# eth-ait/MultiPly

Measured on NVIDIA H100. Metric: rays/sec, higher is better.
Workload: dtype f32 (fp16 hi/lo split tensor-core operands, fp32 accumulate)

## Files before the change

multiply_b200/csrc/mlp_tc.cu:

```cuda
#include "common.cuh"
#include <vector>
#include <mutex>
#include <type_traits>
#include <stdlib.h>

namespace mp {

enum {
  K_SP_PLAIN = 0,
  K_SP_SAVE = 1,
  K_SP_SEED = 2,
  K_FEAT = 3,
  K_BWD = 4,
  K_FINAL_GRAD = 5,
  K_RELU = 6
};
enum {
  F_INJECT_EMB = 1,
  F_SDF_DOT = 2,
  F_SKIP_GRAD = 4,
  F_EXTRA_IN = 8,
  F_RGB_OUT = 16
};
constexpr int kMaxSteps = 24;
constexpr int kSlotBytes = 32768;
constexpr int kRing = 3;
constexpr int kBlobSlots = 170;

struct TcStep {
  int nk;
  int kind;
  int flags;
  int sig;
  const float* bias;
  int slot_off;
  int sc;
  int terms;
};

struct TcProgram {
  int nsteps;
  TcStep step[kMaxSteps];
  const uint4* blob;
  const float* inv_scale;
  int d_in, multires, E, inj_col, n_extra;
  const float* w8row;
  const float* b8;
  const float* Wrgb;
  const float* brgb;
};

struct TcIO : MlpCall {
  float rz;
  char* scratch;
  size_t scratch_per_cta;
};

constexpr int kConsumers = 2;
constexpr int kThreads = 128 * (1 + kConsumers);

constexpr size_t kSigBytes = (size_t)8 * kConsumers * 32 * 128 * 16;
constexpr size_t kFeatBytes = (size_t)kConsumers * 32 * 128 * 16;
constexpr size_t kGeBytes = (size_t)96 * 128 * 4;
constexpr size_t kEmbBytes = (size_t)96 * 128 * 4;
constexpr size_t kScratchPerCta = kSigBytes + kFeatBytes + kGeBytes + kEmbBytes;

constexpr int kABytes = 2 * 4 * 128 * 128;
constexpr int kSmemBytes = kABytes + kRing * kSlotBytes + 256 + 1024;
static_assert(kSmemBytes <= 232448, "shared memory budget of one CTA (227 KB)");

__device__ __forceinline__ uint32_t smem_u32(const void* p) { return (uint32_t)__cvta_generic_to_shared(p); }

__device__ __forceinline__ void mbar_init(uint64_t* bar, uint32_t count) {
  asm volatile("mbarrier.init.shared::cta.b64 [%0], %1;" ::"r"(smem_u32(bar)), "r"(count));
}
__device__ __forceinline__ void mbar_arrive(uint64_t* bar) {
  asm volatile("mbarrier.arrive.shared::cta.b64 _, [%0];" ::"r"(smem_u32(bar)) : "memory");
}
__device__ __forceinline__ void mbar_expect_tx(uint64_t* bar, uint32_t bytes) {
  asm volatile("mbarrier.arrive.expect_tx.shared::cta.b64 _, [%0], %1;" ::"r"(smem_u32(bar)), "r"(bytes) : "memory");
}
__device__ __forceinline__ void mbar_wait(uint64_t* bar, uint32_t parity) {
  asm volatile(
      "{\n"
      ".reg .pred p;\n"
      "WAIT_LOOP:\n"
      "mbarrier.try_wait.parity.shared::cta.b64 p, [%0], %1;\n"
      "@p bra WAIT_DONE;\n"
      "bra WAIT_LOOP;\n"
      "WAIT_DONE:\n"
      "}\n" ::"r"(smem_u32(bar)),
      "r"(parity)
      : "memory");
}
__device__ __forceinline__ void bulk_g2s(void* dst, const void* src, uint32_t bytes, uint64_t* bar) {
  asm volatile("cp.async.bulk.shared::cluster.global.mbarrier::complete_tx::bytes [%0], [%1], %2, [%3];" ::"r"(
                   smem_u32(dst)),
               "l"(src), "r"(bytes), "r"(smem_u32(bar))
               : "memory");
}
__device__ __forceinline__ void prefetch_l2(const void* p, uint32_t bytes) {
  asm volatile("cp.async.bulk.prefetch.L2.global [%0], %1;" ::"l"(p), "r"(bytes) : "memory");
}
__device__ __forceinline__ void fence_async_smem() { asm volatile("fence.proxy.async.shared::cta;" ::: "memory"); }

__device__ __forceinline__ void wg_sync(int id) { asm volatile("bar.sync %0, 128;" ::"r"(id) : "memory"); }

__device__ __forceinline__ void wgmma_fence() { asm volatile("wgmma.fence.sync.aligned;" ::: "memory"); }
__device__ __forceinline__ void wgmma_commit() { asm volatile("wgmma.commit_group.sync.aligned;" ::: "memory"); }
template <int N>
__device__ __forceinline__ void wgmma_wait() {
  asm volatile("wgmma.wait_group.sync.aligned %0;" ::"n"(N) : "memory");
}
__device__ __forceinline__ void acc_fence(float* d) {
#pragma unroll
  for (int i = 0; i < 128; ++i) asm volatile("" : "+f"(d[i])::"memory");
}

#define MP_D4(i) "+f"(d[i]), "+f"(d[i + 1]), "+f"(d[i + 2]), "+f"(d[i + 3])
#define MP_D16(i) MP_D4(i), MP_D4(i + 4), MP_D4(i + 8), MP_D4(i + 12)
__device__ __forceinline__ void wgmma_f16(float* d, uint64_t a_desc, uint64_t b_desc, uint32_t accumulate) {
  asm volatile(
      "{\n"
      ".reg .pred p;\n"
      "setp.ne.b32 p, %130, 0;\n"
      "wgmma.mma_async.sync.aligned.m64n256k16.f32.f16.f16 "
      "{%0, %1, %2, %3, %4, %5, %6, %7, %8, %9, %10, %11, %12, %13, %14, %15, "
      "%16, %17, %18, %19, %20, %21, %22, %23, %24, %25, %26, %27, %28, %29, %30, %31, "
      "%32, %33, %34, %35, %36, %37, %38, %39, %40, %41, %42, %43, %44, %45, %46, %47, "
      "%48, %49, %50, %51, %52, %53, %54, %55, %56, %57, %58, %59, %60, %61, %62, %63, "
      "%64, %65, %66, %67, %68, %69, %70, %71, %72, %73, %74, %75, %76, %77, %78, %79, "
      "%80, %81, %82, %83, %84, %85, %86, %87, %88, %89, %90, %91, %92, %93, %94, %95, "
      "%96, %97, %98, %99, %100, %101, %102, %103, %104, %105, %106, %107, %108, %109, %110, %111, "
      "%112, %113, %114, %115, %116, %117, %118, %119, %120, %121, %122, %123, %124, %125, %126, %127}, "
      "%128, %129, p, 1, 1, 0, 0;\n"
      "}\n"
      : MP_D16(0), MP_D16(16), MP_D16(32), MP_D16(48), MP_D16(64), MP_D16(80), MP_D16(96), MP_D16(112)
      : "l"(a_desc), "l"(b_desc), "r"(accumulate));
}
#undef MP_D16
#undef MP_D4

__device__ __forceinline__ uint64_t make_desc(uint32_t saddr) {
  return (uint64_t)((saddr >> 4) & 0x3FFF) | (1ull << 16) | ((uint64_t)(1024 >> 4) << 32) | (1ull << 62);
}

__device__ __forceinline__ uint32_t a_off(int row, int kb, int ch) {
  return (uint32_t)(kb * 16384 + row * 128 + ((ch ^ (row & 7)) << 4));
}

__device__ __forceinline__ void split2(float a, float b, uint32_t& hi, uint32_t& lo) {
  __half2 h = __floats2half2_rn(a, b);
  float2 f = __half22float2(h);
  __half2 l = __floats2half2_rn(a - f.x, b - f.y);
  hi = *(uint32_t*)&h;
  lo = *(uint32_t*)&l;
}
__device__ __forceinline__ void split8(const float* v, uint4& hi, uint4& lo) {
  split2(v[0], v[1], hi.x, lo.x);
  split2(v[2], v[3], hi.y, lo.y);
  split2(v[4], v[5], hi.z, lo.z);
  split2(v[6], v[7], hi.w, lo.w);
}

__device__ __forceinline__ void sts128(uint32_t A32, uint32_t off, const uint4& v) {
  asm volatile("st.shared.v4.b32 [%0], {%1, %2, %3, %4};" ::"r"(A32 + off), "r"(v.x), "r"(v.y), "r"(v.z), "r"(v.w));
}
__device__ __forceinline__ void store_a8(uint32_t A32, int row, int col, const float* v) {
  uint4 hi, lo;
  split8(v, hi, lo);
  uint32_t o = a_off(row, col >> 6, (col >> 3) & 7);
  sts128(A32, o, hi);
  sts128(A32, 65536 + o, lo);
}
__device__ __forceinline__ void stsm4(uint32_t addr, uint32_t a, uint32_t b, uint32_t c, uint32_t e) {
  asm volatile("stmatrix.sync.aligned.m8n8.x4.shared.b16 [%0], {%1, %2, %3, %4};" ::"r"(addr), "r"(a), "r"(b), "r"(c),
               "r"(e));
}
__device__ __forceinline__ void store_pairs(uint32_t lane_base, uint32_t lane_x, int jp, const uint4& hi, const uint4& lo) {
  const uint32_t addr = lane_base + (uint32_t)(jp >> 2) * 16384u + ((((uint32_t)(2 * jp) & 7u) ^ lane_x) << 4);
  stsm4(addr, hi.x, hi.y, hi.z, hi.w);
  stsm4(addr + 65536u, lo.x, lo.y, lo.z, lo.w);
}
__device__ __forceinline__ void store_acc16(uint32_t lane_base, uint32_t lane_x, int jp, const float* v) {
  uint4 hi, lo;
  split8(v, hi, lo);
  store_pairs(lane_base, lane_x, jp, hi, lo);
}

__device__ __forceinline__ float quad_sum(float v) {
  v += __shfl_xor_sync(0xffffffffu, v, 1);
  v += __shfl_xor_sync(0xffffffffu, v, 2);
  return v;
}

__device__ __forceinline__ float4 ld_stream(const float4* p) {
  float4 v;
  asm volatile("ld.global.cg.v4.f32 {%0,%1,%2,%3}, [%4];" : "=f"(v.x), "=f"(v.y), "=f"(v.z), "=f"(v.w) : "l"(p));
  return v;
}
__device__ __forceinline__ uint4 ld_stream(const uint4* p) {
  uint4 v;
  asm volatile("ld.global.cg.v4.u32 {%0,%1,%2,%3}, [%4];" : "=r"(v.x), "=r"(v.y), "=r"(v.z), "=r"(v.w) : "l"(p));
  return v;
}
__device__ __forceinline__ void st_stream(float4* p, const float4& v) {
  asm volatile("st.global.cg.v4.f32 [%0], {%1,%2,%3,%4};" ::"l"(p), "f"(v.x), "f"(v.y), "f"(v.z), "f"(v.w) : "memory");
}
__device__ __forceinline__ void st_stream(uint4* p, const uint4& v) {
  asm volatile("st.global.cg.v4.u32 [%0], {%1,%2,%3,%4};" ::"l"(p), "r"(v.x), "r"(v.y), "r"(v.z), "r"(v.w) : "memory");
}

__device__ __forceinline__ void discard_line(const void* p, float dep) {
  asm volatile("discard.global.L2 [%0], 128;" ::"l"(p), "f"(dep) : "memory");
}
__device__ __forceinline__ void discard_line(const void* p, uint32_t dep) {
  asm volatile("discard.global.L2 [%0], 128;" ::"l"(p), "r"(dep) : "memory");
}

__device__ __forceinline__ float ex2_approx(float x) {
  float y;
  asm("ex2.approx.ftz.f32 %0, %1;" : "=f"(y) : "f"(x));
  return y;
}
__device__ __forceinline__ float lg2_approx(float x) {
  float y;
  asm("lg2.approx.ftz.f32 %0, %1;" : "=f"(y) : "f"(x));
  return y;
}
__device__ __forceinline__ float rcp_approx(float x) {
  float y;
  asm("rcp.approx.ftz.f32 %0, %1;" : "=f"(y) : "f"(x));
  return y;
}
__device__ __forceinline__ float softplus_fast(float z) {
  float t = z * 144.26950408889634f;
  float u = ex2_approx(t);
  float y = lg2_approx(1.f + u) * 0.0069314718055994531f;
  return t > 28.853900817779268f ? z : y;
}
__device__ __forceinline__ void softplus_fast_grad(float z, float& y, float& d) {
  float t = z * 144.26950408889634f;
  float u = ex2_approx(t);
  float w = 1.f + u;
  float r = rcp_approx(w);
  float ys = lg2_approx(w) * 0.0069314718055994531f;
  bool big = t > 28.853900817779268f;
  y = big ? z : ys;
  d = big ? 1.f : u * r;
}

__device__ __forceinline__ void final_grad(const TcProgram& P, const TcIO& io, const float* acc, float isc, int q,
                                           const float* ge, const float* emb, const int (&rowt)[2],
                                           const bool (&valid)[2], const int (&pt)[2], const int (&slot)[2],
                                           float (&nrm)[2][3]) {
  const int d = P.d_in;
  float gax[2][4] = {{0.f, 0.f, 0.f, 0.f}, {0.f, 0.f, 0.f, 0.f}};
  const int nterm = 1 + 2 * P.multires;
#pragma unroll
  for (int j = 0; j < 8; ++j) {
    if (j < 2 * d) {
      const int a = j >> 1;
#pragma unroll
      for (int e = 0; e < 4; ++e) {
        const int jj = (8 * j + 2 * q + (e & 1)) & 15;
        if (jj < nterm) {
          const int h = e >> 1;
          const int fq = (jj - 1) >> 1;
          const bool is_cos = ((jj - 1) & 1) != 0;
          const int k = (jj == 0) ? a : d + 2 * fq * d + (is_cos ? d : 0) + a;
          const float pg = ge[(size_t)k * 128 + rowt[h]];
          const float tot = fmaf(acc[4 * j + e], isc, pg);
          float w = 1.f;
          if (jj > 0) {
            const float pe = emb[(size_t)(is_cos ? k - d : k + d) * 128 + rowt[h]];
            w = (float)(1 << fq) * (is_cos ? -pe : pe);
          }
          gax[h][a] = fmaf(w, tot, gax[h][a]);
        }
      }
    }
  }
#pragma unroll
  for (int h = 0; h < 2; ++h) {
#pragma unroll
    for (int a = 0; a < 4; ++a) gax[h][a] = quad_sum(gax[h][a]);
    const float gx0 = gax[h][0], gx1 = d > 1 ? gax[h][1] : 0.f, gx2 = d > 2 ? gax[h][2] : 0.f;
    if (q == 0 && io.grad && valid[h]) {
      io.grad[3 * (size_t)pt[h]] = gx0;
      io.grad[3 * (size_t)pt[h] + 1] = gx1;
      io.grad[3 * (size_t)pt[h] + 2] = gx2;
    }
    float n0 = 0.f, n1 = 0.f, n2 = 0.f;
    if (io.jinv && valid[h]) {
      const float4* J4 = (const float4*)(io.jinv + 12 * (size_t)pt[h]);
      const float4 ja = __ldg(J4), jb = __ldg(J4 + 1), jc = __ldg(J4 + 2);
      float v0 = gx0 * ja.x + gx1 * ja.w + gx2 * jb.z;
      float v1 = gx0 * ja.y + gx1 * jb.x + gx2 * jb.w;
      float v2 = gx0 * ja.z + gx1 * jb.y + gx2 * jc.x;
      float nr = fmaxf(sqrtf(v0 * v0 + v1 * v1 + v2 * v2), 1e-12f);
      const float inr = 1.f / nr;
      v0 *= inr; v1 *= inr; v2 *= inr;
      float n2r = fmaxf(sqrtf(v0 * v0 + v1 * v1 + v2 * v2), 1e-6f);
      const float in2 = 1.f / n2r;
      n0 = v0 * in2; n1 = v1 * in2; n2 = v2 * in2;
      if (q == 0 && io.nrm) {
        io.nrm[3 * (size_t)slot[h]] = n0;
        io.nrm[3 * (size_t)slot[h] + 1] = n1;
        io.nrm[3 * (size_t)slot[h] + 2] = n2;
      }
    }
    nrm[h][0] = n0;
    nrm[h][1] = n1;
    nrm[h][2] = n2;
  }
}

__global__ void __launch_bounds__(kThreads, 1) tc_chain_kernel(const __grid_constant__ TcProgram P,
                                                               const __grid_constant__ TcIO io) {
  extern __shared__ uint8_t smem_raw[];
  const int warp = threadIdx.x >> 5, lane = threadIdx.x & 31;
  char* base = (char*)(((uintptr_t)smem_raw + 1023) & ~(uintptr_t)1023);
  char* A = base;
  const uint32_t A32 = smem_u32(A);
  char* ring = base + kABytes;
  uint64_t* bars = (uint64_t*)(ring + kRing * kSlotBytes);
  uint64_t* full = bars;
  uint64_t* empty = bars + kRing;

  const int count = io.count ? min(io.cap, *io.count) : io.cap;
  const int ntiles = (count + 127) >> 7;

  if (threadIdx.x == 0) {
    for (int i = 0; i < kRing; ++i) {
      mbar_init(&full[i], 1);
      mbar_init(&empty[i], 4 * kConsumers);
    }
    asm volatile("fence.mbarrier_init.release.cluster;" ::: "memory");
  }
  __syncthreads();

  if (warp < 4) {
    asm volatile("setmaxnreg.dec.sync.aligned.u32 40;\n" ::: "memory");
    if (warp == 0 && lane == 0) {
      uint32_t it = 0;
      for (int tile = blockIdx.x; tile < ntiles; tile += gridDim.x) {
        for (int s = 0; s < P.nsteps; ++s) {
          const char* src = (const char*)P.blob + (size_t)P.step[s].slot_off * kSlotBytes;
          const int nslot = 2 * P.step[s].nk;
          const int jstep = P.step[s].terms == 1 ? 2 : 1;
          for (int j = 0; j < nslot; j += jstep, ++it) {
            int r = it % kRing;
            uint32_t ph = (it / kRing) & 1;
            mbar_wait(&empty[r], ph ^ 1);
            mbar_expect_tx(&full[r], kSlotBytes);
            bulk_g2s(ring + (size_t)r * kSlotBytes, src + (size_t)j * kSlotBytes, kSlotBytes, &full[r]);
          }
        }
      }
    }
    return;
  }
  asm volatile("setmaxnreg.inc.sync.aligned.u32 232;\n" ::: "memory");
  const int g = (warp >> 2) - 1;
  const int t = threadIdx.x & 127;
  const int wq = warp & 3, q = lane & 3;
  const int bar_id = 1 + g;
  int rowt[2];
  rowt[0] = 64 * g + 16 * wq + (lane >> 2);
  rowt[1] = rowt[0] + 8;
  const int mi = lane >> 3, rr = lane & 7;
  const uint32_t lane_base = A32 + (uint32_t)(64 * g + 16 * wq + 8 * (mi & 1) + rr) * 128u;
  const uint32_t lane_x = (uint32_t)((mi >> 1) ^ rr);
  const uint32_t a_hi = A32 + (uint32_t)g * 8192u, a_lo = a_hi + 65536u;

  char* scr = io.scratch + (size_t)blockIdx.x * io.scratch_per_cta;
  float4* sig = (float4*)scr;
  uint4* fsc = (uint4*)(scr + kSigBytes) + (size_t)g * 32 * 128;
  float* ge = (float*)(scr + kSigBytes + kFeatBytes);
  float* emb = (float*)(scr + kSigBytes + kFeatBytes + kGeBytes);
  const int d = P.d_in, E = P.E;

  float acc[128];
#pragma unroll
  for (int i = 0; i < 128; ++i) acc[i] = 0.f;
  uint32_t it = 0;

  for (int tile = blockIdx.x; tile < ntiles; tile += gridDim.x) {
    int pt[2], slot[2];
    bool valid[2];
    float x[2][4];
#pragma unroll
    for (int h = 0; h < 2; ++h) {
      pt[h] = tile * 128 + rowt[h];
      valid[h] = pt[h] < count;
      for (int a = 0; a < 4; ++a) x[h][a] = 0.f;
      if (valid[h])
        for (int a = 0; a < d; ++a) x[h][a] = io.x[(size_t)pt[h] * d + a];
      slot[h] = valid[h] ? (io.slot ? io.slot[pt[h]] : pt[h]) : 0;
    }
    {
      const int npair = d * P.multires;
      for (int pi = q; pi < npair; pi += 4) {
        const int f = pi / d, a = pi - f * d;
#pragma unroll
        for (int h = 0; h < 2; ++h) {
          float sn, cs;
          sincosf(__fmul_rn(x[h][a], (float)(1 << f)), &sn, &cs);
          emb[(size_t)(d + 2 * f * d + a) * 128 + rowt[h]] = sn;
          emb[(size_t)(d + (2 * f + 1) * d + a) * 128 + rowt[h]] = cs;
        }
      }
      if (q == 0)
        for (int a = 0; a < d; ++a)
#pragma unroll
          for (int h = 0; h < 2; ++h) emb[(size_t)a * 128 + rowt[h]] = x[h][a];
      if (io.dirs) {
        float dv[2][3];
#pragma unroll
        for (int h = 0; h < 2; ++h)
          for (int a = 0; a < 3; ++a) dv[h][a] = valid[h] ? io.dirs[(size_t)pt[h] * 3 + a] : 0.f;
        const int nvp = (P.n_extra - 3) / 2;
        for (int pi = q; pi < nvp; pi += 4) {
          const int f = pi / 3, a = pi - f * 3;
#pragma unroll
          for (int h = 0; h < 2; ++h) {
            float sn, cs;
            sincosf(__fmul_rn(dv[h][a], (float)(1 << f)), &sn, &cs);
            ge[(size_t)(3 + 6 * f + a) * 128 + rowt[h]] = sn;
            ge[(size_t)(3 + 6 * f + 3 + a) * 128 + rowt[h]] = cs;
          }
        }
        if (q == 0)
          for (int a = 0; a < 3; ++a)
#pragma unroll
            for (int h = 0; h < 2; ++h) ge[(size_t)a * 128 + rowt[h]] = dv[h][a];
      }
      __threadfence_block();
      wg_sync(bar_id);
      const int njp = P.step[0].nk * 4;
      for (int jp = 0; jp < njp; ++jp) {
        float v[8];
#pragma unroll
        for (int i = 0; i < 8; ++i) {
          const int c = 16 * jp + 8 * (i >> 2) + 2 * q + (i & 1);
          v[i] = (c < E) ? emb[(size_t)c * 128 + rowt[(i >> 1) & 1]] : 0.f;
        }
        store_acc16(lane_base, lane_x, jp, v);
      }
    }
    float nrm[2][3] = {{0.f, 0.f, 0.f}, {0.f, 0.f, 0.f}};
    for (int s = 0; s < P.nsteps; ++s) {
      const TcStep st = P.step[s];
      const float isc = P.inv_scale[st.sc] * fmaf(io.rz, (float)(4 * st.nk * (st.terms == 1 ? 1 : 3)), 1.f);
      const bool one_term = st.terms == 1;
      if (t == 0) {
        char* ws = io.scratch + (size_t)blockIdx.x * io.scratch_per_cta;
        if (st.kind == K_BWD && st.sig >= 0)
          prefetch_l2(ws + (((size_t)st.sig * kConsumers + g) * 32 * 128) * 16, 32 * 128 * 16);
        if (st.kind == K_FINAL_GRAD) prefetch_l2(ws + kSigBytes + (size_t)g * 32 * 128 * 16, 32 * 128 * 16);
      }

      fence_async_smem();
      wg_sync(bar_id);
      wgmma_fence();
      bool held = false;
      uint32_t held_slot = 0;
      auto release = [&](uint32_t slot_it) {
        if (lane == 0) mbar_arrive(&empty[slot_it % kRing]);
      };
      auto slot_issued = [&](uint32_t slot_it) {
        wgmma_commit();
        if (held) {
          wgmma_wait<1>();
          release(held_slot);
        }
        held = true;
        held_slot = slot_it;
      };
      for (int kc = 0; kc < st.nk; ++kc) {
        if (kc == 4) {
          wgmma_wait<0>();
          acc_fence(acc);
          if (held) release(held_slot);
          held = false;
#pragma unroll
          for (int h = 0; h < 2; ++h) {
#pragma unroll
            for (int c8 = 0; c8 < 16; c8 += 8) {
              const int e0 = 16 * q + c8;
              float xv[8];
#pragma unroll
              for (int j = 0; j < 8; ++j) xv[j] = 0.f;
              if (io.dirs) {
#pragma unroll
                for (int j = 0; j < 8; ++j)
                  if (e0 + j < P.n_extra) xv[j] = ge[(size_t)(e0 + j) * 128 + rowt[h]];
              } else if (e0 == 0) {
                xv[0] = x[h][0]; xv[1] = x[h][1]; xv[2] = x[h][2];
                xv[3] = nrm[h][0]; xv[4] = nrm[h][1]; xv[5] = nrm[h][2];
              }
              store_a8(A32, rowt[h], e0, xv);
            }
          }
          fence_async_smem();
          wg_sync(bar_id);
          wgmma_fence();
        }
        const uint32_t ka = (uint32_t)(kc & 3) * 16384u;
        int r = it % kRing;
        mbar_wait(&full[r], (it / kRing) & 1);
        uint32_t wb = smem_u32(ring + (size_t)r * kSlotBytes);
#pragma unroll
        for (int ks = 0; ks < 4; ++ks) {
          const uint64_t bd = make_desc(wb + ks * 32);
          wgmma_f16(acc, make_desc(a_hi + ka + ks * 32), bd, (kc | ks) != 0);
          if (!one_term) wgmma_f16(acc, make_desc(a_lo + ka + ks * 32), bd, 1);
        }
        slot_issued(it++);
        if (!one_term) {
          r = it % kRing;
          mbar_wait(&full[r], (it / kRing) & 1);
          wb = smem_u32(ring + (size_t)r * kSlotBytes);
#pragma unroll
          for (int ks = 0; ks < 4; ++ks) wgmma_f16(acc, make_desc(a_hi + ka + ks * 32), make_desc(wb + ks * 32), 1);
          slot_issued(it++);
        }
      }
      wgmma_wait<0>();
      acc_fence(acc);
      if (held) release(held_slot);

      auto reload_features = [&]() {
#pragma unroll
        for (int jp = 0; jp < 16; ++jp) {
          const uint4 fh = ld_stream(&fsc[(size_t)jp * 128 + t]);
          const uint4 fl = ld_stream(&fsc[(size_t)(16 + jp) * 128 + t]);
          store_pairs(lane_base, lane_x, jp, fh, fl);
          if ((lane & 7) == 0) {
            discard_line(&fsc[(size_t)jp * 128 + t], fh.x);
            discard_line(&fsc[(size_t)(16 + jp) * 128 + t], fl.x);
          }
        }
      };
      if (st.kind == K_FINAL_GRAD) {
        final_grad(P, io, acc, isc, q, ge, emb, rowt, valid, pt, slot, nrm);
        if (s + 1 < P.nsteps) reload_features();
        continue;
      }

      auto run_epi = [&](auto kind) {
        constexpr int KIND = decltype(kind)::value;
        float dot[2][3] = {{0.f, 0.f, 0.f}, {0.f, 0.f, 0.f}};
#pragma unroll
        for (int jp = 0; jp < 16; ++jp) {
          float* v = acc + 8 * jp;
          float yv[8];
#pragma unroll
          for (int jj = 0; jj < 2; ++jj) {
            const int j = 2 * jp + jj;
            const int c = 8 * j + 2 * q;
            float* u = v + 4 * jj;
            float b[2] = {0.f, 0.f};
            if constexpr (KIND != K_BWD) {
              const float2 b2 = __ldg((const float2*)(st.bias + c));
              b[0] = b2.x;
              b[1] = b2.y;
            }
            if constexpr (KIND == K_SP_SEED) {
              const float2 w2 = __ldg((const float2*)(P.w8row + c));
              const float w[2] = {w2.x, w2.y};
#pragma unroll
              for (int e = 0; e < 4; ++e) {
                float y, dd;
                softplus_fast_grad(fmaf(u[e], isc, b[e & 1]), y, dd);
                dot[e >> 1][0] = fmaf(y, w[e & 1], dot[e >> 1][0]);
                yv[4 * jj + e] = y;
                u[e] = dd * w[e & 1];
              }
            } else if constexpr (KIND == K_SP_SAVE || KIND == K_SP_PLAIN) {
              if constexpr (KIND == K_SP_SAVE) {
                float dd[4];
#pragma unroll
                for (int e = 0; e < 4; ++e) softplus_fast_grad(fmaf(u[e], isc, b[e & 1]), u[e], dd[e]);
                st_stream(&sig[(((size_t)st.sig * kConsumers + g) * 32 + j) * 128 + t], make_float4(dd[0], dd[1], dd[2], dd[3]));
              } else {
#pragma unroll
                for (int e = 0; e < 4; ++e) u[e] = softplus_fast(fmaf(u[e], isc, b[e & 1]));
              }
              if ((st.flags & F_INJECT_EMB) && c + 1 >= P.inj_col) {
#pragma unroll
                for (int e = 0; e < 4; ++e)
                  if (c + (e & 1) >= P.inj_col) u[e] = emb[(size_t)(c + (e & 1) - P.inj_col) * 128 + rowt[e >> 1]];
              }
              if (st.flags & F_SDF_DOT) {
                const float2 w2 = __ldg((const float2*)(P.w8row + c));
                dot[0][0] = fmaf(u[0], w2.x, fmaf(u[1], w2.y, dot[0][0]));
                dot[1][0] = fmaf(u[2], w2.x, fmaf(u[3], w2.y, dot[1][0]));
              }
            } else if constexpr (KIND == K_FEAT) {
#pragma unroll
              for (int e = 0; e < 4; ++e) u[e] = fmaf(u[e], isc, b[e & 1]);
              if (io.feat) {
#pragma unroll
                for (int h = 0; h < 2; ++h)
                  if (valid[h]) *(float2*)(io.feat + (size_t)pt[h] * 256 + c) = make_float2(u[2 * h], u[2 * h + 1]);
              }
            } else if constexpr (KIND == K_BWD) {
              float4 s4 = make_float4(1.f, 1.f, 1.f, 1.f);
              const float4* sp = &sig[(((size_t)(st.sig < 0 ? 0 : st.sig) * kConsumers + g) * 32 + j) * 128 + t];
              if (st.sig >= 0) s4 = ld_stream(sp);
              const float sv[4] = {s4.x, s4.y, s4.z, s4.w};
              if ((st.flags & F_SKIP_GRAD) && c + 1 >= P.inj_col) {
#pragma unroll
                for (int e = 0; e < 4; ++e) {
                  const float gval = u[e] * isc;
                  const int col = c + (e & 1);
                  if (col >= P.inj_col) {
                    ge[(size_t)(col - P.inj_col) * 128 + rowt[e >> 1]] = gval;
                    u[e] = 0.f;
                  } else {
                    u[e] = gval * sv[e];
                  }
                }
              } else {
#pragma unroll
                for (int e = 0; e < 4; ++e) u[e] *= isc * sv[e];
              }
              if (st.sig >= 0 && (lane & 7) == 0) discard_line(sp, s4.x);
            } else {
#pragma unroll
              for (int e = 0; e < 4; ++e) u[e] = fmaxf(fmaf(u[e], isc, b[e & 1]), 0.f);
              if (st.flags & F_RGB_OUT) {
#pragma unroll
                for (int k = 0; k < 3; ++k) {
                  const float2 w2 = __ldg((const float2*)(P.Wrgb + 256 * k + c));
                  dot[0][k] = fmaf(u[0], w2.x, fmaf(u[1], w2.y, dot[0][k]));
                  dot[1][k] = fmaf(u[2], w2.x, fmaf(u[3], w2.y, dot[1][k]));
                }
              }
            }
          }
          if constexpr (KIND == K_SP_SEED) {
            uint4 fh, fl;
            split8(yv, fh, fl);
            st_stream(&fsc[(size_t)jp * 128 + t], fh);
            st_stream(&fsc[(size_t)(16 + jp) * 128 + t], fl);
          }
          bool to_a = true;
          if constexpr (KIND == K_RELU) to_a = !(st.flags & F_RGB_OUT);
          if (to_a) store_acc16(lane_base, lane_x, jp, v);
        }
        if (st.flags & F_SDF_DOT) {
#pragma unroll
          for (int h = 0; h < 2; ++h) {
            const float sdot = quad_sum(dot[h][0]);
            if (q == 0 && valid[h] && io.sdf) io.sdf[slot[h]] = __ldg(P.b8) + sdot;
          }
        }
        if constexpr (KIND == K_RELU) {
          if (st.flags & F_RGB_OUT) {
#pragma unroll
            for (int h = 0; h < 2; ++h) {
#pragma unroll
              for (int k = 0; k < 3; ++k) {
                const float z = __ldg(P.brgb + k) + quad_sum(dot[h][k]);
                if (q == 0 && valid[h] && io.rgb) io.rgb[3 * (size_t)slot[h] + k] = 1.f / (1.f + __expf(-z));
              }
            }
          }
        }
      };
      switch (st.kind) {
        case K_SP_PLAIN: run_epi(std::integral_constant<int, K_SP_PLAIN>{}); break;
        case K_SP_SAVE: run_epi(std::integral_constant<int, K_SP_SAVE>{}); break;
        case K_SP_SEED: run_epi(std::integral_constant<int, K_SP_SEED>{}); break;
        case K_FEAT: run_epi(std::integral_constant<int, K_FEAT>{}); break;
        case K_BWD: run_epi(std::integral_constant<int, K_BWD>{}); break;
        default: run_epi(std::integral_constant<int, K_RELU>{}); break;
      }
      if (st.flags & F_SKIP_GRAD) __threadfence_block();
    }
  }
}

struct TcBlob {
  TcProgram sdf_prog;
  TcProgram full_prog;
  TcProgram fwd_prog;
  bool has_full;
};

__global__ void absmax_kernel(const float* __restrict__ W, int n, float* __restrict__ inv_scale) {
  __shared__ float s[256];
  float m = 0.f;
  for (int i = threadIdx.x; i < n; i += blockDim.x) m = fmaxf(m, fabsf(W[i]));
  s[threadIdx.x] = m;
  __syncthreads();
  for (int o = 128; o > 0; o >>= 1) {
    if (threadIdx.x < o) s[threadIdx.x] = fmaxf(s[threadIdx.x], s[threadIdx.x + o]);
    __syncthreads();
  }
  if (threadIdx.x == 0) {
    float mx = s[0];
    int ex = 0;
    if (mx > 0.f) frexpf(mx, &ex);
    float sc = ldexpf(1.f, 14 - ex);
    inv_scale[0] = 1.f / sc;
  }
}

__global__ void pack_slot_kernel(const float* __restrict__ W, int ld, int transposed, int n_off, int k_off,
                                 int n_valid, int k_valid, int kc, const float* __restrict__ inv_scale,
                                 uint8_t* __restrict__ dst_hi, uint8_t* __restrict__ dst_lo, int perm16) {
  int idx = blockIdx.x * blockDim.x + threadIdx.x;
  if (idx >= 256 * 64) return;
  int n = idx >> 6, k = idx & 63;
  int kk = kc * 64 + k;
  int ns = n;
  if (perm16) {
    const int dd = perm16, a = n >> 4, j = n & 15;
    ns = n_valid;
    if (n < 64 && a < dd) {
      const int k = (j == 0) ? a : dd + ((j - 1) >> 1) * 2 * dd + ((j - 1) & 1) * dd + a;
      if (k < n_valid) ns = k;
    }
  }
  float w = 0.f;
  if (ns < n_valid && kk < k_valid)
    w = transposed ? W[(size_t)(k_off + kk) * ld + n_off + ns] : W[(size_t)(n_off + ns) * ld + k_off + kk];
  w = __fdiv_rn(w, inv_scale[0]);
  __half h = __float2half_rn(w);
  __half l = __float2half_rn(w - __half2float(h));
  uint32_t off = (uint32_t)(n * 128 + ((((k >> 3) ^ (n & 7))) << 4) + (k & 7) * 2);
  *(__half*)(dst_hi + off) = h;
  *(__half*)(dst_lo + off) = l;
}

__global__ void copy_strided_kernel(const float* __restrict__ src, int stride, int n, float* __restrict__ dst) {
  int i = blockIdx.x * blockDim.x + threadIdx.x;
  if (i < n) dst[i] = src[(size_t)i * stride];
}

__global__ void pad_rows_kernel(const float* __restrict__ src, int lds, int nrows, int ncols, float* __restrict__ dst) {
  int i = blockIdx.x * blockDim.x + threadIdx.x;
  if (i >= nrows * 256) return;
  int r = i >> 8, c = i & 255;
  dst[i] = (c < ncols) ? src[(size_t)r * lds + c] : 0.f;
}

__global__ void fold_mm_kernel(const float* __restrict__ Wc, int ldc, int coff, const float* __restrict__ W8f, int ld8,
                               const float* __restrict__ b8f, int n_rows, float* __restrict__ M, int ldm,
                               float* __restrict__ cb) {
  int k = blockIdx.x * 16 + threadIdx.x, n = blockIdx.y * 16 + threadIdx.y;
  if (n >= n_rows || k >= 256) return;
  const float* w = Wc + (size_t)n * ldc + coff;
  double acc = 0.0;
  for (int j = 0; j < 256; ++j) acc += (double)w[j] * (double)W8f[(size_t)j * ld8 + k];
  M[(size_t)n * ldm + k] = (float)acc;
  if (k == 0) {
    double a2 = 0.0;
    for (int j = 0; j < 256; ++j) a2 += (double)w[j] * (double)b8f[j];
    cb[n] = (float)a2;
  }
}

__global__ void fill_extra_cols_kernel(const float* __restrict__ Wt, int n_out, int n_extra, float* __restrict__ M, int ldm) {
  int i = blockIdx.x * blockDim.x + threadIdx.x;
  if (i >= 256 * 64) return;
  int n = i >> 6, e = i & 63;
  M[(size_t)n * ldm + 256 + e] = (n < n_out && e < n_extra) ? Wt[(size_t)e * n_out + n] : 0.f;
}

size_t tc_pack_bytes() { return (size_t)kBlobSlots * kSlotBytes + (1 << 20); }

struct PackCtx {
  cudaStream_t st;
  uint8_t* blob;
  int nslots;
  int nlayers;
  float* inv_scale;
};

static int pack_layer(PackCtx& c, TcStep& stp, int kind, int flags, int sig, const float* bias, const float* W, int ld,
                      int transposed, int n_off, int n_valid, int k_valid, int nk, int total_elems, int perm16 = 0) {
  MP_REQUIRE(c.nslots + 2 * nk <= kBlobSlots, "tc_pack: slot budget exceeded (%d)", c.nslots + 2 * nk);
  const int layer = c.nlayers++;
  stp.nk = nk;
  stp.kind = kind;
  stp.flags = flags;
  stp.sig = sig;
  stp.bias = bias;
  stp.slot_off = c.nslots;
  stp.sc = layer;
  stp.terms = 3;
  absmax_kernel<<<1, 256, 0, c.st>>>(W, total_elems, c.inv_scale + layer);
  MP_LAUNCH_CHECK();
  for (int kc = 0; kc < nk; ++kc) {
    uint8_t* hi = c.blob + (size_t)c.nslots * kSlotBytes;
    uint8_t* lo = hi + kSlotBytes;
    pack_slot_kernel<<<64, 256, 0, c.st>>>(W, ld, transposed, n_off, 0, n_valid, k_valid, kc, c.inv_scale + layer, hi,
                                           lo, perm16);
    MP_LAUNCH_CHECK();
    c.nslots += 2;
  }
  return 0;
}

void tc_free(Field& f) {
  delete (TcBlob*)f.tc;
  f.tc = nullptr;
}

int tc_pack(Field& f, Arena& a, cudaStream_t st) {
  TcBlob* tb = new TcBlob();
  memset(tb, 0, sizeof(*tb));
  f.tc = tb;
  const int E = f.emb_dim;
  PackCtx c;
  c.st = st;
  c.nslots = 0;
  c.nlayers = 0;
  c.blob = (uint8_t*)a.take<uint4>((size_t)kBlobSlots * kSlotBytes / 16);
  c.inv_scale = a.take<float>(32);
  float* w8row = a.take<float>(256);
  float* Wrgb = a.take<float>(3 * 256);
  float* b8feat = a.take<float>(256);
  MP_REQUIRE(a.ok, "tc_pack: storage too small");
  MP_CHECK_CUDA(cudaMemsetAsync(c.blob, 0, (size_t)kBlobSlots * kSlotBytes, st));
  TcProgram P;
  memset(&P, 0, sizeof(P));
  P.blob = (const uint4*)c.blob;
  P.inv_scale = c.inv_scale;
  P.d_in = f.d_in;
  P.multires = f.multires;
  P.E = E;
  P.inj_col = kHidden - E;
  P.w8row = w8row;
  P.b8 = f.imp_b[8];
  P.Wrgb = Wrgb;
  P.n_extra = f.ren_extra;
  copy_strided_kernel<<<1, 256, 0, st>>>(f.imp_W[8], 1, 256, w8row);
  MP_LAUNCH_CHECK();
  copy_strided_kernel<<<1, 256, 0, st>>>(f.imp_b[8] + 1, 1, 256, b8feat);
  MP_LAUNCH_CHECK();
  int s = 0;
  for (int l = 0; l < 8; ++l) {
    const int in = f.imp_in[l], out = f.imp_out[l];
    const int flags = ((l == f.skip_layer - 1) ? F_INJECT_EMB : 0) | ((l == 7) ? F_SDF_DOT : 0);
    MP_TRY(pack_layer(c, P.step[s++], K_SP_PLAIN, flags, l, (l == 0) ? f.imp_b0_eff : f.imp_b[l], f.imp_W[l], in, 0,
                      0, out, (l == 0) ? E : in, (l == 0) ? (E + 63) / 64 : 4, out * in));
  }
  P.nsteps = s;
  tb->sdf_prog = P;
  tb->fwd_prog = P;
  MP_TRY(pack_layer(c, tb->fwd_prog.step[s], K_FEAT, 0, -1, b8feat, f.imp_W[8], 256, 0, 1, 256, 256, 4, 257 * 256));
  tb->fwd_prog.nsteps = s + 1;
  const bool fg_chain = (f.ren_mode == 0) && (f.n_ren == 5) && f.ren_out[0] == 256;
  const bool bg_chain = (f.ren_mode == 1) && (f.n_ren == 2) && f.ren_out[0] <= 256 && f.ren_extra <= 27;
  tb->has_full = fg_chain || bg_chain;
  constexpr int kLdM = 320;
  float* Mfold = a.take<float>(256 * kLdM);
  f.ren_cb = a.take<float>(264);
  f.ren_b0_fold = a.take<float>(264);
  MP_REQUIRE(a.ok, "tc_pack: storage too small");
  if (tb->has_full) {
    const int in0 = f.ren_in[0] == 0 ? 0 : (f.ren_mode == 0 ? 6 + 8 + 256 : f.ren_extra + 32 + 256);
    const int coff = f.ren_mode == 0 ? 14 : f.ren_extra + 32;
    const int o0 = f.ren_out[0];
    fold_mm_kernel<<<dim3(256 / 16, div_up(o0, 16)), dim3(16, 16), 0, st>>>(f.ren_W[0], in0, coff, f.imp_W[8] + 256, 256,
                                                                          f.imp_b[8] + 1, o0, Mfold, kLdM, f.ren_cb);
    MP_LAUNCH_CHECK();
    MP_REQUIRE(f.ren_extra <= 64, "tc_pack: more than 64 extra colour inputs");
    fill_extra_cols_kernel<<<64, 256, 0, st>>>(f.ren_Wt[0], o0, f.ren_extra, Mfold, kLdM);
    MP_LAUNCH_CHECK();
  }
  if (bg_chain) {
    const int o0 = f.ren_out[0];
    MP_TRY(pack_layer(c, P.step[s++], K_RELU, F_EXTRA_IN | F_RGB_OUT, -1, f.ren_b0_fold, Mfold, kLdM, 0, 0, o0, kLdM, 5,
                      256 * kLdM));
    pad_rows_kernel<<<div_up(3 * 256, 256), 256, 0, st>>>(f.ren_W[1], o0, 3, o0, Wrgb);
    MP_LAUNCH_CHECK();
    P.brgb = f.ren_b[1];
    P.nsteps = s;
    tb->full_prog = P;
  }
  if (fg_chain) {
    for (int l = 0; l < 8; ++l) P.step[l].kind = (l == 7) ? K_SP_SEED : K_SP_SAVE;
    for (int l = 7; l >= 1; --l) {
      const int in = f.imp_in[l], out = f.imp_out[l];
      MP_TRY(pack_layer(c, P.step[s++], K_BWD, (l == f.skip_layer) ? F_SKIP_GRAD : 0, l - 1, nullptr, f.imp_W[l], in, 1,
                        0, in, out, 4, out * in));
    }
    MP_REQUIRE(f.d_in <= 4 && 1 + 2 * f.multires <= 14,
               "tc_pack: the final-gradient step keeps 1 + 2 * multires <= 14 embedding columns per axis");
    MP_TRY(pack_layer(c, P.step[s++], K_FINAL_GRAD, 0, -1, nullptr, f.imp_W[0], f.imp_in[0], 1, 0, E, 256, 4,
                      256 * f.imp_in[0], f.d_in));
    MP_TRY(pack_layer(c, P.step[s++], K_RELU, F_EXTRA_IN, -1, f.ren_b0_fold, Mfold, kLdM, 0, 0, 256, kLdM, 5,
                      256 * kLdM));
    for (int l = 1; l < 4; ++l)
      MP_TRY(pack_layer(c, P.step[s++], K_RELU, (l == 3) ? F_RGB_OUT : 0, -1, f.ren_b[l], f.ren_W[l], 256, 0, 0, 256,
                        256, 4, 256 * 256));
    MP_CHECK_CUDA(cudaMemcpyAsync(Wrgb, f.ren_W[4], (size_t)3 * 256 * sizeof(float), cudaMemcpyDeviceToDevice, st));
    P.brgb = f.ren_b[4];
    P.nsteps = s;
    tb->full_prog = P;
  }
  return 0;
}

size_t tc_workspace_bytes(int N) { return (size_t)sm_count() * kScratchPerCta + 4096; }

struct ProfEntry {
  cudaEvent_t e0, e1;
  int kind;
  int cap;
  int* host_count;
};
static std::mutex g_prof_mu;
static std::atomic<bool> g_prof_on{false};
static std::vector<ProfEntry>* g_prof = nullptr;
static int* g_prof_pinned = nullptr;
static int g_prof_used = 0;
constexpr int kProfMax = 1 << 16;

int prof_enable(int on) {
  std::lock_guard<std::mutex> g(g_prof_mu);
  if (on && !g_prof) {
    g_prof = new std::vector<ProfEntry>();
    MP_CHECK_CUDA(cudaMallocHost(&g_prof_pinned, kProfMax * sizeof(int)));
  }
  g_prof_on = on != 0;
  return 0;
}
int prof_read(double* ms, long long* launches, double* points, int reset) {
  for (int k = 0; k < 4; ++k) {
    ms[k] = 0;
    launches[k] = 0;
    points[k] = 0;
  }
  std::lock_guard<std::mutex> g(g_prof_mu);
  if (!g_prof) return 0;
  for (auto& e : *g_prof) {
    MP_CHECK_CUDA(cudaEventSynchronize(e.e1));
    float t = 0.f;
    MP_CHECK_CUDA(cudaEventElapsedTime(&t, e.e0, e.e1));
    ms[e.kind] += t;
    launches[e.kind] += 1;
    int n = e.host_count ? *e.host_count : e.cap;
    points[e.kind] += (double)(n < e.cap ? n : e.cap);
  }
  if (reset) {
    for (auto& e : *g_prof) {
      cudaEventDestroy(e.e0);
      cudaEventDestroy(e.e1);
    }
    g_prof->clear();
    g_prof_used = 0;
  }
  return 0;
}

std::atomic<int> g_precision{0};

constexpr float kRzPerMma = 1.72e-8f;

static int tc_launch(const TcProgram& P0, TcIO io, void* ws, size_t ws_bytes, cudaStream_t st, MlpProg kind) {
  TcProgram P = P0;
  {
    const int mode = g_precision.load();
    for (int s = 0; s < P.nsteps; ++s)
      P.step[s].terms = (mode == 2 || (mode == 1 && P.step[s].kind == K_RELU)) ? 1 : 3;
  }
  int grid = sm_count();
  {
    static int grid_override = -1;
    if (grid_override < 0) {
      const char* eg = getenv("MP_TC_GRID");
      grid_override = eg ? atoi(eg) : 0;
    }
    if (grid_override > 0 && grid_override < grid) grid = grid_override;
  }
  int maxtiles = (io.cap + 127) / 128;
  if (grid > maxtiles) grid = maxtiles;
  if (grid < 1) return 0;
  MP_REQUIRE(ws && ws_bytes >= (size_t)grid * kScratchPerCta, "tensor-core engine: workspace too small (%zu < %zu)",
             ws_bytes, (size_t)grid * kScratchPerCta);
  io.scratch = (char*)ws;
  io.scratch_per_cta = kScratchPerCta;
  static const float rz_scale = [] {
    const char* er = getenv("MP_TC_RZ_SCALE");
    return er ? (float)atof(er) : 1.f;
  }();
  io.rz = kRzPerMma * rz_scale;
  {
    static std::mutex attr_mu;
    static unsigned long long attr_done = 0;
    int dev = 0;
    MP_CHECK_CUDA(cudaGetDevice(&dev));
    std::lock_guard<std::mutex> g(attr_mu);
    if (dev < 0 || dev >= 64 || !((attr_done >> dev) & 1ull)) {
      MP_CHECK_CUDA(cudaFuncSetAttribute(tc_chain_kernel, cudaFuncAttributeMaxDynamicSharedMemorySize, kSmemBytes));
      if (dev >= 0 && dev < 64) attr_done |= 1ull << dev;
    }
  }
  ProfEntry pe;
  std::unique_lock<std::mutex> prof_lock(g_prof_mu, std::defer_lock);
  if (g_prof_on.load()) prof_lock.lock();
  const bool prof = prof_lock.owns_lock() && g_prof_on.load() && g_prof && g_prof_used < kProfMax;
  if (prof) {
    MP_CHECK_CUDA(cudaEventCreate(&pe.e0));
    MP_CHECK_CUDA(cudaEventCreate(&pe.e1));
    pe.kind = (int)kind;
    pe.cap = io.cap;
    pe.host_count = nullptr;
    if (io.count) {
      pe.host_count = g_prof_pinned + g_prof_used++;
      MP_CHECK_CUDA(cudaMemcpyAsync(pe.host_count, io.count, sizeof(int), cudaMemcpyDeviceToHost, st));
    }
    MP_CHECK_CUDA(cudaEventRecord(pe.e0, st));
  }
  tc_chain_kernel<<<grid, kThreads, kSmemBytes, st>>>(P, io);
  MP_LAUNCH_CHECK();
  if (prof) {
    MP_CHECK_CUDA(cudaEventRecord(pe.e1, st));
    g_prof->push_back(pe);
  }
  return 0;
}

int tc_run(const Field& f, const MlpCall& c, void* ws, size_t ws_bytes, cudaStream_t st) {
  MP_REQUIRE(f.tc, "tensor-core engine: field not packed");
  const TcBlob& tb = *(const TcBlob*)f.tc;
  const MlpProg prog = mlp_prog(c);
  TcIO io{};
  static_cast<MlpCall&>(io) = c;
  if (prog == MlpProg::kSdf) return tc_launch(tb.sdf_prog, io, ws, ws_bytes, st, prog);
  if (prog == MlpProg::kForward) return tc_launch(tb.fwd_prog, io, ws, ws_bytes, st, prog);
  if (prog == MlpProg::kBg) {
    MP_REQUIRE(tb.has_full && f.ren_mode == 1, "tensor-core engine: not a background field");
    return tc_launch(tb.full_prog, io, ws, ws_bytes, st, prog);
  }
  MP_REQUIRE(tb.has_full, "tensor-core engine: this field has no fused shading program");
  if (c.feat) {
    TcIO fio{};
    fio.x = c.x;
    fio.slot = c.slot;
    fio.count = c.count;
    fio.cap = c.cap;
    fio.feat = c.feat;
    MP_TRY(tc_launch(tb.fwd_prog, fio, ws, ws_bytes, st, MlpProg::kForward));
    io.feat = nullptr;
  }
  return tc_launch(tb.full_prog, io, ws, ws_bytes, st, prog);
}

}
```

Before: 446,900.

## Split weight slots into 32-wide K halves with 64B swizzle and deeper ring

Halves each TMA weight slot to 16KB, splitting every 64-wide K chunk into two 32-wide halves stored with a 64-byte swizzle layout and a matching B descriptor. The ring depth doubles from 3 to 6 so the same shared memory holds finer-grained stages, letting wgmma start after a smaller transfer and release buffers sooner. It also templates the MMA loop on one_term so that branch is resolved at compile time. Costs are more mbarrier waits and arrivals per chunk, and the repacking and new descriptor must match exactly or results will be wrong.

After: 456,400, median of 6. +2.1%, better.

```diff
diff --git a/multiply_b200/csrc/mlp_tc.cu b/multiply_b200/csrc/mlp_tc.cu
--- a/multiply_b200/csrc/mlp_tc.cu
+++ b/multiply_b200/csrc/mlp_tc.cu
@@ -23,9 +23,9 @@
   F_RGB_OUT = 16
 };
 constexpr int kMaxSteps = 24;
-constexpr int kSlotBytes = 32768;
-constexpr int kRing = 3;
-constexpr int kBlobSlots = 170;
+constexpr int kSlotBytes = 16384;
+constexpr int kRing = 6;
+constexpr int kBlobSlots = 340;
 
 struct TcStep {
   int nk;
@@ -144,6 +144,9 @@
 __device__ __forceinline__ uint64_t make_desc(uint32_t saddr) {
   return (uint64_t)((saddr >> 4) & 0x3FFF) | (1ull << 16) | ((uint64_t)(1024 >> 4) << 32) | (1ull << 62);
 }
+__device__ __forceinline__ uint64_t make_desc_b(uint32_t saddr) {
+  return (uint64_t)((saddr >> 4) & 0x3FFF) | (1ull << 16) | ((uint64_t)(512 >> 4) << 32) | (2ull << 62);
+}
 
 __device__ __forceinline__ uint32_t a_off(int row, int kb, int ch) {
   return (uint32_t)(kb * 16384 + row * 128 + ((ch ^ (row & 7)) << 4));
@@ -347,11 +350,13 @@
       for (int tile = blockIdx.x; tile < ntiles; tile += gridDim.x) {
         for (int s = 0; s < P.nsteps; ++s) {
           const char* src = (const char*)P.blob + (size_t)P.step[s].slot_off * kSlotBytes;
-          const int nslot = 2 * P.step[s].nk;
-          const int jstep = P.step[s].terms == 1 ? 2 : 1;
-          for (int j = 0; j < nslot; j += jstep, ++it) {
-            int r = it % kRing;
-            uint32_t ph = (it / kRing) & 1;
+          const int nslot = 4 * P.step[s].nk;
+          const int nhalf = P.step[s].terms == 1 ? 2 : 4;
+          for (int j = 0; j < nslot; ++j) {
+            if ((j & 3) >= nhalf) continue;
+            const int r = it % kRing;
+            const uint32_t ph = (it / kRing) & 1;
+            ++it;
             mbar_wait(&empty[r], ph ^ 1);
             mbar_expect_tx(&full[r], kSlotBytes);
             bulk_g2s(ring + (size_t)r * kSlotBytes, src + (size_t)j * kSlotBytes, kSlotBytes, &full[r]);
@@ -478,6 +483,8 @@
         held = true;
         held_slot = slot_it;
       };
+      auto mma_chunks = [&](auto one_term_c) {
+      constexpr bool one_term = decltype(one_term_c)::value;
       for (int kc = 0; kc < st.nk; ++kc) {
         if (kc == 4) {
           wgmma_wait<0>();
@@ -508,25 +515,39 @@
           wgmma_fence();
         }
         const uint32_t ka = (uint32_t)(kc & 3) * 16384u;
-        int r = it % kRing;
-        mbar_wait(&full[r], (it / kRing) & 1);
-        uint32_t wb = smem_u32(ring + (size_t)r * kSlotBytes);
-#pragma unroll
-        for (int ks = 0; ks < 4; ++ks) {
-          const uint64_t bd = make_desc(wb + ks * 32);
-          wgmma_f16(acc, make_desc(a_hi + ka + ks * 32), bd, (kc | ks) != 0);
-          if (!one_term) wgmma_f16(acc, make_desc(a_lo + ka + ks * 32), bd, 1);
-        }
-        slot_issued(it++);
-        if (!one_term) {
-          r = it % kRing;
+        auto wait_slot = [&]() {
+          const int r = it % kRing;
           mbar_wait(&full[r], (it / kRing) & 1);
-          wb = smem_u32(ring + (size_t)r * kSlotBytes);
-#pragma unroll
-          for (int ks = 0; ks < 4; ++ks) wgmma_f16(acc, make_desc(a_hi + ka + ks * 32), make_desc(wb + ks * 32), 1);
+          return smem_u32(ring + (size_t)r * kSlotBytes);
+        };
+#pragma unroll
+        for (int hf = 0; hf < 2; ++hf) {
+          const uint32_t wb = wait_slot();
+#pragma unroll
+          for (int ks = 0; ks < 2; ++ks) {
+            const uint64_t bd = make_desc_b(wb + ks * 32);
+            const uint32_t ak = ka + (uint32_t)(2 * hf + ks) * 32u;
+            wgmma_f16(acc, make_desc(a_hi + ak), bd, (kc | hf | ks) != 0);
+            if constexpr (!one_term) wgmma_f16(acc, make_desc(a_lo + ak), bd, 1);
+          }
           slot_issued(it++);
         }
+        if constexpr (!one_term) {
+#pragma unroll
+          for (int hf = 0; hf < 2; ++hf) {
+            const uint32_t wb = wait_slot();
+#pragma unroll
+            for (int ks = 0; ks < 2; ++ks)
+              wgmma_f16(acc, make_desc(a_hi + ka + (uint32_t)(2 * hf + ks) * 32u), make_desc_b(wb + ks * 32), 1);
+            slot_issued(it++);
+          }
+        }
       }
+      };
+      if (one_term)
+        mma_chunks(std::true_type{});
+      else
+        mma_chunks(std::false_type{});
       wgmma_wait<0>();
       acc_fence(acc);
       if (held) release(held_slot);
@@ -732,7 +753,7 @@
   w = __fdiv_rn(w, inv_scale[0]);
   __half h = __float2half_rn(w);
   __half l = __float2half_rn(w - __half2float(h));
-  uint32_t off = (uint32_t)(n * 128 + ((((k >> 3) ^ (n & 7))) << 4) + (k & 7) * 2);
+  uint32_t off = (uint32_t)((k >> 5) * kSlotBytes + n * 64 + ((((k >> 3) & 3) ^ ((n >> 1) & 3)) << 4) + (k & 7) * 2);
   *(__half*)(dst_hi + off) = h;
   *(__half*)(dst_lo + off) = l;
 }
@@ -784,7 +805,7 @@
 
 static int pack_layer(PackCtx& c, TcStep& stp, int kind, int flags, int sig, const float* bias, const float* W, int ld,
                       int transposed, int n_off, int n_valid, int k_valid, int nk, int total_elems, int perm16 = 0) {
-  MP_REQUIRE(c.nslots + 2 * nk <= kBlobSlots, "tc_pack: slot budget exceeded (%d)", c.nslots + 2 * nk);
+  MP_REQUIRE(c.nslots + 4 * nk <= kBlobSlots, "tc_pack: slot budget exceeded (%d)", c.nslots + 4 * nk);
   const int layer = c.nlayers++;
   stp.nk = nk;
   stp.kind = kind;
@@ -798,11 +819,11 @@
   MP_LAUNCH_CHECK();
   for (int kc = 0; kc < nk; ++kc) {
     uint8_t* hi = c.blob + (size_t)c.nslots * kSlotBytes;
-    uint8_t* lo = hi + kSlotBytes;
+    uint8_t* lo = hi + 2 * kSlotBytes;
     pack_slot_kernel<<<64, 256, 0, c.st>>>(W, ld, transposed, n_off, 0, n_valid, k_valid, kc, c.inv_scale + layer, hi,
                                            lo, perm16);
     MP_LAUNCH_CHECK();
-    c.nslots += 2;
+    c.nslots += 4;
   }
   return 0;
 }
```

## Split weight ring slots into N-halves and use m64n128 wgmma for finer pipelining

Applied to the files above, without the earlier changes.

Each 32 KB weight slot is split into two 16 KB halves, the TMA ring grows from 3 to 6 half-slots, and each half feeds m64n128k16 wgmma on one half of the accumulator instead of a single m64n256k16. The aim is finer-grained producer/consumer overlap, so compute can start on the first half while the second is still loading and slots are released sooner. The cost is twice as many wgmma instructions, mbarrier waits and commits. The diff also assumes the blob's slot layout splits cleanly into N-halves, which it does not show.

Measured after the change: 447,500 before, 457,500 after (median of 6 runs). 2.2% higher.

```diff
diff --git a/multiply_b200/csrc/mlp_tc.cu b/multiply_b200/csrc/mlp_tc.cu
--- a/multiply_b200/csrc/mlp_tc.cu
+++ b/multiply_b200/csrc/mlp_tc.cu
@@ -24,7 +24,8 @@
 };
 constexpr int kMaxSteps = 24;
 constexpr int kSlotBytes = 32768;
-constexpr int kRing = 3;
+constexpr int kHalfBytes = kSlotBytes / 2;
+constexpr int kRing = 6;
 constexpr int kBlobSlots = 170;
 
 struct TcStep {
@@ -66,7 +67,7 @@
 constexpr size_t kScratchPerCta = kSigBytes + kFeatBytes + kGeBytes + kEmbBytes;
 
 constexpr int kABytes = 2 * 4 * 128 * 128;
-constexpr int kSmemBytes = kABytes + kRing * kSlotBytes + 256 + 1024;
+constexpr int kSmemBytes = kABytes + kRing * kHalfBytes + 256 + 1024;
 static_assert(kSmemBytes <= 232448, "shared memory budget of one CTA (227 KB)");
 
 __device__ __forceinline__ uint32_t smem_u32(const void* p) { return (uint32_t)__cvta_generic_to_shared(p); }
@@ -123,19 +124,15 @@
   asm volatile(
       "{\n"
       ".reg .pred p;\n"
-      "setp.ne.b32 p, %130, 0;\n"
-      "wgmma.mma_async.sync.aligned.m64n256k16.f32.f16.f16 "
+      "setp.ne.b32 p, %66, 0;\n"
+      "wgmma.mma_async.sync.aligned.m64n128k16.f32.f16.f16 "
       "{%0, %1, %2, %3, %4, %5, %6, %7, %8, %9, %10, %11, %12, %13, %14, %15, "
       "%16, %17, %18, %19, %20, %21, %22, %23, %24, %25, %26, %27, %28, %29, %30, %31, "
       "%32, %33, %34, %35, %36, %37, %38, %39, %40, %41, %42, %43, %44, %45, %46, %47, "
-      "%48, %49, %50, %51, %52, %53, %54, %55, %56, %57, %58, %59, %60, %61, %62, %63, "
-      "%64, %65, %66, %67, %68, %69, %70, %71, %72, %73, %74, %75, %76, %77, %78, %79, "
-      "%80, %81, %82, %83, %84, %85, %86, %87, %88, %89, %90, %91, %92, %93, %94, %95, "
-      "%96, %97, %98, %99, %100, %101, %102, %103, %104, %105, %106, %107, %108, %109, %110, %111, "
-      "%112, %113, %114, %115, %116, %117, %118, %119, %120, %121, %122, %123, %124, %125, %126, %127}, "
-      "%128, %129, p, 1, 1, 0, 0;\n"
+      "%48, %49, %50, %51, %52, %53, %54, %55, %56, %57, %58, %59, %60, %61, %62, %63}, "
+      "%64, %65, p, 1, 1, 0, 0;\n"
       "}\n"
-      : MP_D16(0), MP_D16(16), MP_D16(32), MP_D16(48), MP_D16(64), MP_D16(80), MP_D16(96), MP_D16(112)
+      : MP_D16(0), MP_D16(16), MP_D16(32), MP_D16(48)
       : "l"(a_desc), "l"(b_desc), "r"(accumulate));
 }
 #undef MP_D16
@@ -324,7 +321,7 @@
   char* A = base;
   const uint32_t A32 = smem_u32(A);
   char* ring = base + kABytes;
-  uint64_t* bars = (uint64_t*)(ring + kRing * kSlotBytes);
+  uint64_t* bars = (uint64_t*)(ring + kRing * kHalfBytes);
   uint64_t* full = bars;
   uint64_t* empty = bars + kRing;
 
@@ -347,14 +344,16 @@
       for (int tile = blockIdx.x; tile < ntiles; tile += gridDim.x) {
         for (int s = 0; s < P.nsteps; ++s) {
           const char* src = (const char*)P.blob + (size_t)P.step[s].slot_off * kSlotBytes;
-          const int nslot = 2 * P.step[s].nk;
-          const int jstep = P.step[s].terms == 1 ? 2 : 1;
-          for (int j = 0; j < nslot; j += jstep, ++it) {
+          const int nhalf = 4 * P.step[s].nk;
+          const bool one_term = P.step[s].terms == 1;
+          for (int j = 0; j < nhalf; ++j) {
+            if (one_term && (j & 2)) continue;
             int r = it % kRing;
             uint32_t ph = (it / kRing) & 1;
             mbar_wait(&empty[r], ph ^ 1);
-            mbar_expect_tx(&full[r], kSlotBytes);
-            bulk_g2s(ring + (size_t)r * kSlotBytes, src + (size_t)j * kSlotBytes, kSlotBytes, &full[r]);
+            mbar_expect_tx(&full[r], kHalfBytes);
+            bulk_g2s(ring + (size_t)r * kHalfBytes, src + (size_t)j * kHalfBytes, kHalfBytes, &full[r]);
+            ++it;
           }
         }
       }
@@ -465,24 +464,24 @@
       wg_sync(bar_id);
       wgmma_fence();
       bool held = false;
-      uint32_t held_slot = 0;
-      auto release = [&](uint32_t slot_it) {
-        if (lane == 0) mbar_arrive(&empty[slot_it % kRing]);
+      uint32_t held_half = 0;
+      auto release = [&](uint32_t half_it) {
+        if (lane == 0) mbar_arrive(&empty[half_it % kRing]);
       };
-      auto slot_issued = [&](uint32_t slot_it) {
+      auto half_issued = [&](uint32_t half_it) {
         wgmma_commit();
         if (held) {
           wgmma_wait<1>();
-          release(held_slot);
+          release(held_half);
         }
         held = true;
-        held_slot = slot_it;
+        held_half = half_it;
       };
       for (int kc = 0; kc < st.nk; ++kc) {
         if (kc == 4) {
           wgmma_wait<0>();
           acc_fence(acc);
-          if (held) release(held_slot);
+          if (held) release(held_half);
           held = false;
 #pragma unroll
           for (int h = 0; h < 2; ++h) {
@@ -508,28 +507,42 @@
           wgmma_fence();
         }
         const uint32_t ka = (uint32_t)(kc & 3) * 16384u;
-        int r = it % kRing;
-        mbar_wait(&full[r], (it / kRing) & 1);
-        uint32_t wb = smem_u32(ring + (size_t)r * kSlotBytes);
-#pragma unroll
-        for (int ks = 0; ks < 4; ++ks) {
-          const uint64_t bd = make_desc(wb + ks * 32);
-          wgmma_f16(acc, make_desc(a_hi + ka + ks * 32), bd, (kc | ks) != 0);
-          if (!one_term) wgmma_f16(acc, make_desc(a_lo + ka + ks * 32), bd, 1);
-        }
-        slot_issued(it++);
+        auto next_half = [&]() {
+          const int r = it % kRing;
+          mbar_wait(&full[r], (it / kRing) & 1);
+          return smem_u32(ring + (size_t)r * kHalfBytes);
+        };
+        auto hi_half = [&](float* dn, uint32_t wb, auto three_terms) {
+#pragma unroll
+          for (int ks = 0; ks < 4; ++ks) {
+            const uint64_t bd = make_desc(wb + ks * 32);
+            wgmma_f16(dn, make_desc(a_hi + ka + ks * 32), bd, (kc | ks) != 0);
+            if constexpr (decltype(three_terms)::value) wgmma_f16(dn, make_desc(a_lo + ka + ks * 32), bd, 1);
+          }
+        };
+#pragma unroll
+        for (int nh = 0; nh < 2; ++nh) {
+          const uint32_t wb = next_half();
+          if (one_term)
+            hi_half(acc + 64 * nh, wb, std::false_type{});
+          else
+            hi_half(acc + 64 * nh, wb, std::true_type{});
+          half_issued(it++);
+        }
         if (!one_term) {
-          r = it % kRing;
-          mbar_wait(&full[r], (it / kRing) & 1);
-          wb = smem_u32(ring + (size_t)r * kSlotBytes);
-#pragma unroll
-          for (int ks = 0; ks < 4; ++ks) wgmma_f16(acc, make_desc(a_hi + ka + ks * 32), make_desc(wb + ks * 32), 1);
-          slot_issued(it++);
+#pragma unroll
+          for (int nh = 0; nh < 2; ++nh) {
+            const uint32_t wb = next_half();
+#pragma unroll
+            for (int ks = 0; ks < 4; ++ks)
+              wgmma_f16(acc + 64 * nh, make_desc(a_hi + ka + ks * 32), make_desc(wb + ks * 32), 1);
+            half_issued(it++);
+          }
         }
       }
       wgmma_wait<0>();
       acc_fence(acc);
-      if (held) release(held_slot);
+      if (held) release(held_half);
 
       auto reload_features = [&]() {
 #pragma unroll
```
